# joshloyal/dynetlsm

Measured on AMD Instinct MI355X. Metric: Gibbs iterations/sec (and ms/log-lik eval), T=10 N=2000 d=2, higher is better.
Workload: dtype f64; 1 GPU; DynamicNetworkLSM synthetic undirected T=10 N=2000 d=2, 1 chain per GPU; chains=1, chains_per_gpu=1, sweep_algo=4, network_broadcast=none

## Files before the change

dynetlsm_amd/csrc/capi.hip:

```cpp
#include <hip/hip_runtime.h>
#include <hip/hip_ext.h>

#include <algorithm>
#include <atomic>
#include <cmath>
#include <cstdio>
#include <cstring>
#include <string>
#include <vector>

#include "chain.hpp"
#include "device_common.hpp"
#include "kernels_labels.hpp"
#include "kernels_hdp.hpp"
#include "cc_rows.hpp"
#include "kernels_loglik.hpp"
#include "kernels_loglik_ccstream.hpp"
#include "kernels_hdploop.hpp"
#include "kernels_sweep.hpp"
#include "kernels_dirloop.hpp"
#include "kernels_spec.hpp"
#include "kernels_spec_sweep.hpp"
#include "kernels_spec_pipe.hpp"
#include "kernels_tail_propose.hpp"
#include "kernels_ccpipe.hpp"
#include "kernels_init.hpp"
#include "kernels_post.hpp"
#include "kernels_forecast.hpp"
#include "kernels_forecast_paths.hpp"
#include "kernels_gof.hpp"
#include "kernels_gof_dynamic.hpp"
#include "kernels_ic.hpp"
#include "kernels_score.hpp"
#include "kernels_missing.hpp"
#include "host_draws.hpp"

using namespace dlsm;

static thread_local std::string g_err;
static int32_t *g_fix_err_host = nullptr;
static int g_fix_err_device = -1;
static std::atomic<int> g_live_chains{0};

namespace {

int env_int(const char *name, int unset) { const char *e = getenv(name); return e ? atoi(e) : unset; }
bool env_is(const char *name, const char *word) { const char *e = getenv(name); return e && strcmp(e, word) == 0; }

struct Knobs {
    bool cc_pass_records, cc_pass_rows;
    bool pipe_lds;
    int pipe_xserve, pipe_xbudget;
    int cc_helpers, cc_helper_budget;
    int spec_s;
    bool post_ride, post_fuse, tail_propose, hdp_head;
    bool graph;
    int hdp_queues, hdp_fork_budget;
    bool hdp_gate_kernel;
    bool profiler;
};

Knobs read_knobs() {
    Knobs k;
    k.cc_pass_records = env_is("DLSM_CC_PASS", "records"); k.cc_pass_rows = env_is("DLSM_CC_PASS", "rows");
    k.pipe_lds = env_int("DLSM_PIPE_LDS", 1) != 0;
    k.pipe_xserve = env_int("DLSM_PIPE_XSERVE", 1); k.pipe_xbudget = env_int("DLSM_PIPE_XBUDGET", 1 << 22);
    k.cc_helpers = env_int("DLSM_CC_HELPERS", 1); k.cc_helper_budget = env_int("DLSM_CC_HELPER_BUDGET", 1 << 22);
    k.spec_s = env_int("DLSM_SPEC_S", 2);
    k.post_ride = env_int("DLSM_POST_RIDE", 1) != 0; k.post_fuse = env_int("DLSM_POST_FUSE", 1) != 0;
    k.tail_propose = env_int("DLSM_TAIL_PROPOSE", 1) != 0; k.hdp_head = env_int("DLSM_HDP_HEAD", 1) != 0;
    k.graph = env_int("DLSM_GRAPH", 0) == 1;
    k.hdp_queues = env_int("DLSM_HDP_QUEUES", 0); k.hdp_fork_budget = env_int("DLSM_HDP_FORK_BUDGET", 1 << 22);
    k.hdp_gate_kernel = env_is("DLSM_HDP_GATE", "kernel");
    k.profiler = getenv("ROCP_TOOL_LIBRARIES") != nullptr || getenv("ROCPROFILER_REGISTER_FORCE_LOAD") != nullptr;
    return k;
}

bool labels_wave_forced() {
    static const bool v = env_is("DLSM_LABELS_KERNEL", "wave");
    return v;
}

bool alone_or_forced(int mode, int off, int forced) {
    return mode != off && (mode == forced || g_live_chains.load() == 1);
}

struct Call {
    hipStream_t stream;
    Knobs knobs;
};

struct SweepCall : Call {
    explicit SweepCall(const Call &c) : Call(c) {}
    bool want_post_ride = false; const double *xref = nullptr;
    bool draw_intercept = false, head_only = false, alloc_only = false;
    bool rode = false; int nwg = 0, jl = -1, par = 0;
    bool left_proposals = false;
};

}

#define FAIL(h, code, ...)                                      \
    do {                                                        \
        char _b[512];                                           \
        snprintf(_b, sizeof(_b), __VA_ARGS__);                  \
        if (h) (h)->err = _b; else g_err = _b;                  \
        return (code);                                          \
    } while (0)

#define HIPCHK(h, call)                                                          \
    do {                                                                         \
        hipError_t _e = (call);                                                  \
        if (_e != hipSuccess)                                                    \
            FAIL(h, DLSM_E_HIP, "%s failed: %s (%s:%d)", #call,                  \
                 hipGetErrorString(_e), __FILE__, __LINE__);                     \
    } while (0)

#define NEED(h, cond, ...)                               \
    do {                                                 \
        if (!(cond)) FAIL(h, DLSM_E_ARG, __VA_ARGS__);   \
    } while (0)

#ifdef DLSM_DEV_ONLY_D2
#define DISPATCH_D(h, D_, ...)                                              \
    switch (D_) {                                                           \
        case 2: { constexpr int DD = 2; __VA_ARGS__; } break;               \
        default: FAIL(h, DLSM_E_LIMIT, "n_features=%d: this development build holds n_features = 2 only", D_); \
    }
#else
#define DISPATCH_D(h, D_, ...)                                              \
    switch (D_) {                                                           \
        case 1: { constexpr int DD = 1; __VA_ARGS__; } break;               \
        case 2: { constexpr int DD = 2; __VA_ARGS__; } break;               \
        case 3: { constexpr int DD = 3; __VA_ARGS__; } break;               \
        case 4: { constexpr int DD = 4; __VA_ARGS__; } break;               \
        case 5: { constexpr int DD = 5; __VA_ARGS__; } break;               \
        case 6: { constexpr int DD = 6; __VA_ARGS__; } break;               \
        case 7: { constexpr int DD = 7; __VA_ARGS__; } break;               \
        case 8: { constexpr int DD = 8; __VA_ARGS__; } break;               \
        default: FAIL(h, DLSM_E_LIMIT, "n_features=%d unsupported (1..8)", D_); \
    }
#endif

static int check_pipe_err(dlsm_chain *h);
static int check_sweep_algo(dlsm_chain *h, int algo);
static int build_colmajor(dlsm_chain *h);

static void drop_graph(dlsm_chain *h) {
    if (h->graph_exec) hipGraphExecDestroy(h->graph_exec);
    if (h->graph) hipGraphDestroy(h->graph);
    h->graph_exec = nullptr; h->graph = nullptr; h->graph_ref = -2; h->graph_algo = -1;
}

namespace {

struct ProfScope {
    dlsm_chain *h; int k; hipStream_t q; hipEvent_t e0 = nullptr, e1 = nullptr;
    ProfScope(dlsm_chain *h_, int k_) : ProfScope(h_, k_, h_->stream) {}
    ProfScope(dlsm_chain *h_, int k_, hipStream_t q_) : h(h_), k(k_), q(q_) {
        if (h->profiling) {
            hipEventCreate(&e0); hipEventCreate(&e1);
            hipEventRecord(e0, q);
        }
    }
    ~ProfScope() {
        if (h->profiling) {
            hipEventRecord(e1, q);
            h->prof[k].pending.emplace_back(e0, e1);
        }
    }
};

template <typename T>
int dev_alloc(dlsm_chain *h, T **p, size_t n) {
    HIPCHK(h, hipMalloc((void **)p, std::max<size_t>(n, 1) * sizeof(T)));
    return DLSM_OK;
}

constexpr size_t STAGE_BYTES = 256 * 1024;
constexpr size_t STAGE_D2H_MAX = 64 * 1024;

template <typename T>
int h2d(dlsm_chain *h, T *dst, const T *src, size_t n) {
    const size_t bytes = n * sizeof(T);
    const void *from = src;
    if (h->stage && bytes <= STAGE_BYTES) { memcpy(h->stage, src, bytes); from = h->stage; }
    HIPCHK(h, hipMemcpyAsync(dst, from, bytes, hipMemcpyHostToDevice, h->stream));
    HIPCHK(h, hipStreamSynchronize(h->stream));
    return DLSM_OK;
}

template <typename T>
int d2h(dlsm_chain *h, T *dst, const T *src, size_t n) {
    const size_t bytes = n * sizeof(T);
    const bool staged = h->stage && bytes <= STAGE_D2H_MAX;
    HIPCHK(h, hipMemcpyAsync(staged ? h->stage : (void *)dst, src, bytes, hipMemcpyDeviceToHost,
                             h->stream));
    HIPCHK(h, hipStreamSynchronize(h->stream));
    if (staged) memcpy(dst, h->stage, bytes);
    return DLSM_OK;
}

template <typename T>
int h2d_enqueue(dlsm_chain *h, T *dst, const T *src, size_t n, size_t *off) {
    const size_t bytes = n * sizeof(T);
    const void *from = src;
    if (h->stage && *off + bytes <= STAGE_BYTES) {
        from = (char *)h->stage + *off;
        memcpy((void *)from, src, bytes);
        *off += (bytes + 255) & ~(size_t)255;
    }
    HIPCHK(h, hipMemcpyAsync(dst, from, bytes, hipMemcpyHostToDevice, h->stream));
    return DLSM_OK;
}

int upload_i64_as_i32(dlsm_chain *h, int32_t **dst, const int64_t *src, size_t n,
                      int64_t lo, int64_t hi, const char *what) {
    std::vector<int32_t> tmp(n);
// ... 777 lines not shown
    const size_t TN = (size_t)h->T * h->N;
    rc = ensure_partials(h, TN); if (rc) return rc;
    DISPATCH_D(h, h->D, rc = launch_partial<DD>(h, with_prior, -1, -1, nullptr, h->partials));
    if (rc) return rc;
    return d2h(h, out, h->partials, TN);
}

}


template <int DD, int SBM>
static void launch_spec_eval(dlsm_chain *h, const ChainView &v, const SpecBuf &sg, dim3 grid,
                             hipStream_t q, int parity, int j0, int nsb) {
    hipEvent_t e0 = nullptr, e1 = nullptr;
    if (h->profiling) { hipEventCreate(&e0); hipEventCreate(&e1); }
    if (h->model == DLSM_UNDIRECTED)
        hipExtLaunchKernelGGL((k_spec_eval<DD, DLSM_UNDIRECTED, SBM>), grid, dim3(SP_EV_THREADS),
                              0, q, e0, e1, 0, v, sg, parity, j0, nsb);
    else
        hipExtLaunchKernelGGL((k_spec_eval<DD, DLSM_DIRECTED, SBM>), grid, dim3(SP_EV_THREADS),
                              0, q, e0, e1, 0, v, sg, parity, j0, nsb);
    if (h->profiling) h->prof[DLSM_K_SWEEP_EVAL].pending.emplace_back(e0, e1);
}

template <int DD>
static int launch_sweep_spec(dlsm_chain *h, const SweepCall &sc, IterRef iter, int S) {
    const int N = h->N, T = h->T;
    hipStream_t q = sc.stream;
    if (h->model == DLSM_DIRECTED_CASE_CONTROL) S = 1;
    S = std::max(1, std::min(S, SP_SMAX));
    const int B = std::min(S * SP_BMAX, (N + 1) / 2 * 2);
    const int nsl_max = (T + 1) / 2;
    int parts = (1024 + nsl_max * SP_BMAX - 1) / (nsl_max * SP_BMAX);
    parts = std::max(1, std::min(parts, 8));
    if (h->model == DLSM_DIRECTED_CASE_CONTROL) parts = 1;
    auto even2 = [](size_t n) { return (n + 1) / 2 * 2; };
    const size_t n_full0 = even2((size_t)nsl_max * B * parts);
    const size_t n_prop = even2((size_t)nsl_max * N * (DD + 2));
    const size_t n_ht = (size_t)nsl_max * B * B;
    const size_t need = (n_full0 + n_prop + n_ht + 2) * sizeof(double);
    if (h->spec_cap < need) {
        if (h->spec) hipFree(h->spec);
        h->spec = nullptr; h->spec_cap = 0;
        HIPCHK(h, hipMalloc((void **)&h->spec, need));
        h->spec_cap = need;
    }
    SpecBuf sb;
    sb.full0 = h->spec; sb.prop = sb.full0 + n_full0; sb.Ht = sb.prop + n_prop;
    sb.consts = sb.Ht + n_ht;
    sb.B = B; sb.parts = parts; sb.s0 = 0; sb.per = (N + parts - 1) / parts;
    sb.stamps = nullptr;
    ChainView v = h->view();
    auto resolve = k_spec_resolve<DD>;
    const size_t lds = (size_t)SP_BMAX * SP_BMAX * sizeof(double);
    HIPCHK(h, hipFuncSetAttribute((const void *)resolve,
                                  hipFuncAttributeMaxDynamicSharedMemorySize, (int)lds));
    if (sc.alloc_only) return DLSM_OK;
    for (int parity = 0; parity < 2; ++parity) {
        const int nsl = (T - parity + 1) / 2;
        if (nsl <= 0) continue;
        hipLaunchKernelGGL((k_spec_propose<DD>), dim3((N + 255) / 256, nsl), dim3(256), 0, q, v, sb, iter, parity);
        for (int j0 = 0; j0 < N; j0 += B) {
            const int nsb = std::min(B, N - j0);
            SpecBuf sg = sb;
            const size_t nblk = (size_t)parts * nsb * nsl;
            if (h->profiling && h->stamps && h->model != DLSM_DIRECTED_CASE_CONTROL &&
                h->stamps_used + nblk <= h->stamps_cap) {
                sg.stamps = h->stamps + 2 * h->stamps_used;
                h->stamp_launches.emplace_back(h->stamps_used, nblk);
                h->stamps_used += nblk;
            }
            if (h->model == DLSM_DIRECTED_CASE_CONTROL) {
                ProfScope pe(h, DLSM_K_SWEEP_EVAL, q);
                hipLaunchKernelGGL((k_spec_eval_cc<DD>), dim3((unsigned)(nsl * nsb)),
                                   dim3(64), 0, q, v, sg, h->nctrl, parity, j0, nsb);
            } else if (S == 1)
                launch_spec_eval<DD, SP_BMAX>(h, v, sg, dim3(parts, nsb, nsl), q, parity, j0, nsb);
            else if (S == 2)
                launch_spec_eval<DD, 2 * SP_BMAX>(h, v, sg, dim3(parts, nsb, nsl), q, parity, j0, nsb);
            else
                launch_spec_eval<DD, SP_SMAX * SP_BMAX>(h, v, sg, dim3(parts, nsb, nsl), q, parity, j0, nsb);
            {
                ProfScope pr(h, DLSM_K_SWEEP_RESOLVE, q);
                hipLaunchKernelGGL(resolve, dim3(nsl), dim3(SP_RES_THREADS), lds, q, v, sg, parity, j0, nsb);
            }
        }
    }
    HIPCHK(h, hipGetLastError());
    return DLSM_OK;
}


static int resolve_sweep_algo(const dlsm_chain *h, int algo) {
    if (algo != 0) return algo;
    if (h->D > DLSM_D_PIPE_MAX) return h->N >= 256 ? 2 : 1;
    if (h->model == DLSM_DIRECTED_CASE_CONTROL)
        return (h->N >= 2048 && h->D <= DLSM_D_CCPIPE_MAX) ? 5 : (h->N >= 512 ? 4 : (h->N >= 256 ? 2 : 1));
    return h->N >= 512 ? 4 : (h->N >= 256 ? 2 : 1);
}

template <int DD, int MODEL, int G = 1>
static void launch_pipe_step(dlsm_chain *h, hipStream_t q, const ChainView &v, const PipeBuf &pb, dim3 grid,
                             size_t lds, int l) {
    hipEvent_t e0 = nullptr, e1 = nullptr;
    if (h->profiling) { hipEventCreate(&e0); hipEventCreate(&e1); }
    hipExtLaunchKernelGGL((k_pipe_step<DD, MODEL, G>), grid, dim3(PP_THREADS), lds, q,
                          e0, e1, 0, v, pb, l);
    if (h->profiling) h->prof[DLSM_K_SWEEP_EVAL].pending.emplace_back(e0, e1);
}

static int check_pipe_err(dlsm_chain *h) {
    if (g_fix_err_host && *(volatile int32_t *)g_fix_err_host != 0) {
        const int32_t e = *(volatile int32_t *)g_fix_err_host;
        *(volatile int32_t *)g_fix_err_host = 0;
        FAIL(h, DLSM_E_HIP, "case-control sweep: a resolver's fixed point did not settle inside its spin bound "
             "(word %#x) - the state of this process's case-control chains is undefined; set it again", e);
    }
    if (h->fork_err_host) {
        const int32_t e = *(volatile int32_t *)h->fork_err_host;
        if (e != 0) {
            *(volatile int32_t *)h->fork_err_host = 0;
            if (e & PP_ERR_XSERVE)
                FAIL(h, DLSM_E_HIP, "pipelined sweep: a resolver ran out of its poll budget waiting for a cross product "
                     "from the launch's evaluators (word %#x) - the chain's state is undefined; set the state again "
                     "and run with DLSM_PIPE_XSERVE=0", e);
            if (e & CC_ERR_HELPER)
                FAIL(h, DLSM_E_HIP, "case-control sweep: a resolver ran out of its poll budget waiting for its helper "
                     "workgroup (word %#x) - the chain's state is undefined; set the state again and run with "
                     "DLSM_CC_HELPERS=0", e);
            FAIL(h, DLSM_E_HIP, "HDP-LPCM loop: a hand-over between the chain's two queues ran out of its poll "
                 "budget (flags %d) - the chain's state is undefined (more streams alive than hardware "
                 "queues?); set the state again and run with DLSM_HDP_QUEUES=1", e);
        }
    }
    return DLSM_OK;
}

template <int DD>
static int launch_sweep_pipe(dlsm_chain *h, SweepCall &sc, IterRef iter) {
    constexpr int G = 1;
    hipStream_t q = sc.stream;
    const Knobs &kn = sc.knobs;
    const int N = h->N, T = h->T;
    const int nbat = (N + PP_B - 1) / PP_B;
    const bool cc = h->model == DLSM_DIRECTED_CASE_CONTROL;
    int ne_wg = std::max(h->n_cu / 2, h->n_cu - T);
    int parts = (int)((double)ne_wg * PP_WAVES / ((double)T * PP_B) + 0.5);
    parts = std::max(1, std::min(parts, PP_MAXPARTS));
    if (h->model == DLSM_UNDIRECTED && parts > 1 && (long)parts * T * PP_B > (long)ne_wg * PP_WAVES) --parts;
    if (cc) {
        parts = CC_PARTS;
        ne_wg = std::min(ne_wg, (T * PP_B * CC_PARTS + PP_WAVES - 1) / PP_WAVES);
    }
    auto even2 = [](size_t n) { return (n + 1) / 2 * 2; };
    const size_t n_prop = even2((size_t)T * N * (2 * DD + 2));
    const int xr = (2 * G - 1) * PP_B;
    const size_t n_full0 = (size_t)2 * G * T * PP_B * parts * 2;
    const size_t n_h = (size_t)2 * G * T * PP_B * PP_B;
    const size_t n_hx = (size_t)2 * G * T * xr * PP_B;
    const size_t n_acc = even2(((size_t)T * 2 * G * PP_ACC + 1) / 2);
    const size_t n_xp = (size_t)T * PP_B;
    const size_t need = (n_prop + n_full0 + n_h + n_hx + n_acc + 2 + n_xp) * sizeof(double);
    if (h->pipe_cap < need) {
        if (h->pipe) hipFree(h->pipe);
        h->pipe = nullptr; h->pipe_cap = 0;
        HIPCHK(h, hipMalloc((void **)&h->pipe, need));
        h->pipe_cap = need;
    }
    PipeBuf pb{};
    pb.prop = h->pipe; pb.full0 = pb.prop + n_prop; pb.Hd = pb.full0 + n_full0;
    pb.Hx = pb.Hd + n_h; pb.acc = (int32_t *)(pb.Hx + n_hx);
    pb.consts = pb.Hx + n_hx + n_acc;
    pb.xprod = pb.consts + 2;
    pb.sync = nullptr; pb.nsync = 0; pb.queue0 = ne_wg;
    pb.lsm_draw = sc.draw_intercept ? h->lsm : nullptr;
    pb.parts = parts; pb.nbat = nbat;
    pb.G = G; pb.xr = xr;
    pb.per = ((N + parts - 1) / parts + 63) / 64 * 64;
    pb.nctrl = h->nctrl;
    const size_t lds = (size_t)PP_B * PR_LD * sizeof(double);
    pb.lds_eval = h->model == DLSM_UNDIRECTED && pipe_lds_eval_bytes(N, DD, parts) <= lds &&
                  (long)parts * T * PP_B <= (long)ne_wg * PP_WAVES && kn.pipe_lds;
    pb.err = h->fork_err_dev;
    pb.budget = kn.pipe_xbudget;
    const int xserve_sweep = pb.lds_eval && pb.err != nullptr && T < 128 && alone_or_forced(kn.pipe_xserve, 0, 2);
    pb.xserve = 0;
    ChainView v = h->view();
    {
        PipeLds &a = pb.lds;
        a.X = v.X; a.ybits = v.ybits; a.prop = pb.prop; a.full0 = pb.full0; a.Hd = pb.Hd; a.acc = pb.acc;
        a.consts = pb.consts; a.xprod = pb.xprod;
        a.T = T; a.N = N; a.W = v.W; a.squared = v.squared; a.parts = parts; a.nbat = nbat;
        a.lds_cap = pipe_lds_trip_cap((N + 63) / 64, parts); a.xserve = 0;
    }
    for (int nw = 1; nw <= 4; ++nw)
        for (int p = 0; p < PP_MAXPARTS; ++p)
            pb.lds.plan[nw - 1][p] = p < parts ? pipe_plan_entry((N + 63) / 64, parts, nw, p) : 0u;
    auto ku = k_pipe_step<DD, DLSM_UNDIRECTED>;
    auto kl = k_pipe_step<DD, PIPE_UNDIRECTED_LONG>;
    auto kd = k_pipe_step<DD, DLSM_DIRECTED>;
    auto kc = k_pipe_step<DD, DLSM_DIRECTED_CASE_CONTROL>;
    HIPCHK(h, hipFuncSetAttribute((const void *)ku, hipFuncAttributeMaxDynamicSharedMemorySize,
                                  (int)lds));
    HIPCHK(h, hipFuncSetAttribute((const void *)kl, hipFuncAttributeMaxDynamicSharedMemorySize,
                                  (int)lds));
    HIPCHK(h, hipFuncSetAttribute((const void *)kd, hipFuncAttributeMaxDynamicSharedMemorySize,
                                  (int)lds));
    HIPCHK(h, hipFuncSetAttribute((const void *)kc, hipFuncAttributeMaxDynamicSharedMemorySize,
                                  (int)lds));
    HIPCHK(h, hipFuncSetAttribute((const void *)k_pipe_last_ride<DD>,
                                  hipFuncAttributeMaxDynamicSharedMemorySize, (int)lds));
    if (sc.alloc_only) return DLSM_OK;
    {
        const ProposeBuf nb{pb.prop, pb.consts, pb.sync, pb.nsync, pb.queue0, pb.lsm_draw};
        if (!h->carry.drawn(iter.ptr ? -1L : (long)iter.value, nb))
            hipLaunchKernelGGL((k_pipe_propose<DD>), dim3((N + 255) / 256, T), dim3(256), 0, q, v, pb, iter);
        h->carry.taken(nb); sc.left_proposals = true;
    }
    const int nlaunch = (nbat + G - 1) / G;
    const int last = T > 1 ? nlaunch : nlaunch - 1;
    for (int l = -1; l <= last; ++l) {
        if (l == -1 && !iter.ptr && h->carry.head_done_for == (long)iter.value) continue;
        if (sc.head_only && l >= 0) break;
        const bool any_eval = (G * (l + 1) < nbat) || (T > 1 && l >= 0 && G * l < nbat);
        const int grid = T + (any_eval ? ne_wg : 0);
        const bool lng = !pb.lds_eval;
        if (l == last && !any_eval && sc.want_post_ride && G == 1 && h->model == DLSM_UNDIRECTED &&
            !h->profiling && l >= 0 && T + 4 <= PS_BLOCKS) {
            const long rows = (long)T * N;
            const int nwg = (int)std::min<long>(PS_BLOCKS - T, (rows + PP_THREADS - 1) / PP_THREADS);
            PipePostRide pr{sc.xref, iter, h->partials + (size_t)ll_blocks(h) * 4, nwg,
                            (nbat - 1) * PP_B, T > 1 ? 1 : 0};
            hipLaunchKernelGGL((k_pipe_last_ride<DD>), dim3(T + nwg), dim3(PP_THREADS), lds, q, v, pb, l, pr);
            sc.rode = true; sc.nwg = nwg + T; sc.jl = pr.jl; sc.par = pr.par;
            continue;
        }
        if (h->model == DLSM_UNDIRECTED && lng)
            launch_pipe_step<DD, PIPE_UNDIRECTED_LONG>(h, q, v, pb, dim3(grid), lds, l);
        else if (h->model == DLSM_UNDIRECTED && pb.lds_eval && any_eval) {
            const int beE = l + 1, beO = l, nE = (T + 1) / 2, nO = T / 2;
            PipeLds &a = pb.lds;
            a.beE = beE; a.beO = beO;
            a.nbE = (beE >= 0 && beE < nbat) ? std::min(PP_B, N - beE * PP_B) : 0;
            a.nbO = (beO >= 0 && beO < nbat) ? std::min(PP_B, N - beO * PP_B) : 0;
            a.nslE = a.nbE > 0 ? nE : 0; a.nslO = a.nbO > 0 ? nO : 0;
            const int gx = PP_B / PP_WAVES, nsl = a.nslE + a.nslO;
            a.nsl_magic = (65536u + (uint32_t)nsl - 1u) / (uint32_t)nsl;
            a.xstride = (T * PP_B + ne_wg - 1) / ne_wg;
            pb.xserve = a.xserve = xserve_sweep && a.xstride <= PP_WAVES;
            (void)gx;
            launch_pipe_step<DD, DLSM_UNDIRECTED>(h, q, v, pb, dim3(grid), lds, l);
        } else if (h->model == DLSM_UNDIRECTED)
            launch_pipe_step<DD, DLSM_UNDIRECTED>(h, q, v, pb, dim3(grid), lds, l);
        else if (h->model == DLSM_DIRECTED)
            launch_pipe_step<DD, DLSM_DIRECTED>(h, q, v, pb, dim3(grid), lds, l);
        else
            launch_pipe_step<DD, DLSM_DIRECTED_CASE_CONTROL>(h, q, v, pb, dim3(grid), lds, l);
    }
    HIPCHK(h, hipGetLastError());
    return DLSM_OK;
}

template <int DD>
static int launch_sweep_ccpipe(dlsm_chain *h, SweepCall &sc, IterRef iter) {
    hipStream_t q = sc.stream;
    const int N = h->N, T = h->T;
    const int nbat = (N + CP_B - 1) / CP_B;
    const int cap = std::max(1, h->Din + h->Dout + 2 * h->C);
    auto even2 = [](size_t n) { return (n + 1) / 2 * 2; };
    const size_t n_prop = even2((size_t)T * N * (2 * DD + 2));
    const size_t n_tot = (size_t)2 * T * CP_B;
    const size_t n_ent = (size_t)2 * T * cap * CP_B;
    const size_t n_cnt = (size_t)2 * T * CP_B * 2;
    const size_t n_rec = (size_t)T * N * cp_record_width(DD);
    const size_t n_xsum = (size_t)T * CP_B;
    const size_t need = (n_prop + n_tot + 2 * n_ent + 2 + 2 * n_rec + n_xsum) * sizeof(double) +
                        even2(2 * n_ent + n_cnt) * sizeof(int32_t) +
                        (size_t)T * CP_WAVES * sizeof(unsigned long long);
    if (h->pipe_cap < need) {
        if (h->pipe) hipFree(h->pipe);
        h->pipe = nullptr; h->pipe_cap = 0;
        HIPCHK(h, hipMalloc((void **)&h->pipe, need));
        h->pipe_cap = need;
    }
    if (N >= (1 << 24) || (double)(T + 1) * N * cp_record_width(DD) * sizeof(double) >= 4294967296.0)
        FAIL(h, DLSM_E_LIMIT, "case-control sweep (algo 5): N=%d T=%d is beyond its 32-bit gather offsets "
             "(N < 2^24, (T + 1) N record bytes < 2^32); use sweep_algo 4 or 2", N, T);
    { int rc_ = ensure_cc_rows(h, q, sc.alloc_only); if (rc_) return rc_; }
    const int tw = h->cc_tw;
    if (sc.alloc_only) return DLSM_OK;
    CcPipeBuf pb;
    pb.prop = h->pipe; pb.tot = pb.prop + n_prop; pb.xval = pb.tot + n_tot; pb.oval = pb.xval + n_ent;
    double *consts = pb.oval + n_ent;
    pb.cur = consts + 2; pb.snap = pb.cur + n_rec;
    pb.xsum = pb.snap + n_rec;
    pb.xidx = (int32_t *)(pb.xsum + n_xsum); pb.oidx = pb.xidx + n_ent; pb.cnt = pb.oidx + n_ent;
    pb.accmask = (unsigned long long *)(pb.xidx + even2(2 * n_ent + n_cnt));
    pb.helpers = alone_or_forced(sc.knobs.cc_helpers, 0, 2) && h->n_cu >= 4 * T && h->fork_err_dev != nullptr;
    pb.budget = sc.knobs.cc_helper_budget;
    pb.err = h->fork_err_dev;
    pb.nctrl = h->nctrl; pb.cap = cap; pb.nbat = nbat;
    pb.terms = h->cc_terms; pb.tw = tw;
    PipeBuf pp{};
    pp.prop = pb.prop; pp.consts = consts;
    ChainView v = h->view();
    {
        const ProposeBuf nb{pp.prop, pp.consts, nullptr, 0, 0, nullptr};
        if (!h->carry.drawn(iter.ptr ? -1L : (long)iter.value, nb))
            hipLaunchKernelGGL((k_pipe_propose<DD>), dim3((N + 255) / 256, T), dim3(256), 0, q, v, pp, iter);
        h->carry.taken(nb); sc.left_proposals = true;
    }
    hipLaunchKernelGGL((k_ccpipe_pack<DD>), dim3((unsigned)(((size_t)T * N + 255) / 256)), dim3(256), 0,
                       q, v, pb);
    const int nodes_max = ((T + 1) / 2 + T / 2) * std::min(CP_B, N);
    const int n_front = pb.helpers ? 2 * T : T;
    const int ne_wg = std::max(1, std::min(std::max(h->n_cu / 2, h->n_cu - n_front), nodes_max));
    const int last = T > 1 ? nbat : nbat - 1;
    for (int l = -1; l <= last; ++l) {
        const bool any_eval = (l + 1 < nbat) || (T > 1 && l >= 0 && l < nbat);
        const int grid = n_front + (any_eval ? ne_wg : 0);
        hipEvent_t e0 = nullptr, e1 = nullptr;
        if (h->profiling) { hipEventCreate(&e0); hipEventCreate(&e1); }
        hipExtLaunchKernelGGL((k_ccpipe_step<DD>), dim3(grid), dim3(CP_THREADS), 0, q, e0, e1,
                              0, v, pb, l);
        if (h->profiling) h->prof[DLSM_K_SWEEP_EVAL].pending.emplace_back(e0, e1);
    }
    HIPCHK(h, hipGetLastError());
    return DLSM_OK;
}

template <int DD>
static int launch_sweep(dlsm_chain *h, SweepCall &sc, IterRef iter, int algo) {
    ChainView v = h->view();
    hipStream_t q = sc.stream;
    const bool alloc_only = sc.alloc_only;
    ProfScope ps(h, DLSM_K_SWEEP, q);
    if (h->model == DLSM_DIRECTED_CASE_CONTROL) {
        { int rc_ = ensure_cc_rows(h, q, alloc_only); if (rc_) return rc_; }
        algo = resolve_sweep_algo(h, algo);
        if (alloc_only) hipStreamSynchronize(q);
        if constexpr (DD <= DLSM_D_CCPIPE_MAX) {
            if (algo == 5) return launch_sweep_ccpipe<DD>(h, sc, iter);
        }
        if constexpr (DD <= DLSM_D_PIPE_MAX) {
            if (algo == 4) return launch_sweep_pipe<DD>(h, sc, iter);
        }
        if (algo >= 2) return launch_sweep_spec<DD>(h, sc, iter, 1);
        if (alloc_only) return DLSM_OK;
        for (int parity = 0; parity < 2; ++parity) {
            int nsl = (h->T - parity + 1) / 2;
            if (nsl <= 0) continue;
            hipLaunchKernelGGL((k_sweep_casecontrol<DD>), dim3(nsl), dim3(CC_THREADS), 0,
                               q, v, h->nctrl, iter, parity);
        }
        HIPCHK(h, hipGetLastError());
        return DLSM_OK;
    }
    algo = resolve_sweep_algo(h, algo);
    if constexpr (DD <= DLSM_D_PIPE_MAX) {
        if (algo == 4) return launch_sweep_pipe<DD>(h, sc, iter);
    }
    if (algo == 2) return launch_sweep_spec<DD>(h, sc, iter, 1);
    if (algo == 3) return launch_sweep_spec<DD>(h, sc, iter, sc.knobs.spec_s);
    const size_t lds = sweep_slice_lds_bytes(h->N, DD, h->W, h->model);
    if (lds > 160 * 1024)
        FAIL(h, DLSM_E_LIMIT, "N=%d needs %zu B of LDS in the slice sweep (max 163840)",
             h->N, lds);
    {
        auto ku = k_sweep_slice<DD, DLSM_UNDIRECTED>;
        auto kd = k_sweep_slice<DD, DLSM_DIRECTED>;
        HIPCHK(h, hipFuncSetAttribute((const void *)ku,
                                      hipFuncAttributeMaxDynamicSharedMemorySize, (int)lds));
        HIPCHK(h, hipFuncSetAttribute((const void *)kd,
                                      hipFuncAttributeMaxDynamicSharedMemorySize, (int)lds));
    }
    if (alloc_only) return DLSM_OK;
    for (int parity = 0; parity < 2; ++parity) {
        int nsl = (h->T - parity + 1) / 2;
        if (nsl <= 0) continue;
        if (h->model == DLSM_UNDIRECTED)
            hipLaunchKernelGGL((k_sweep_slice<DD, DLSM_UNDIRECTED>), dim3(nsl), dim3(SW_THREADS),
                               lds, q, v, iter, parity);
        else
            hipLaunchKernelGGL((k_sweep_slice<DD, DLSM_DIRECTED>), dim3(nsl), dim3(SW_THREADS),
                               lds, q, v, iter, parity);
    }
    HIPCHK(h, hipGetLastError());
    return DLSM_OK;
}

static int check_sweep_algo(dlsm_chain *h, int algo) {
    NEED(h, algo >= 0 && algo <= 5, "algo must be 0..5 (6 and 7, measured slower than 4, were removed in round 5)");
    NEED(h, algo != 5 || h->model == DLSM_DIRECTED_CASE_CONTROL, "algo 5 is the case-control sweep");
    NEED(h, algo != 4 || h->D <= DLSM_D_PIPE_MAX, "the pipelined sweep (algo 4) is built for n_features <= 8");
    NEED(h, algo != 5 || h->D <= DLSM_D_CCPIPE_MAX,
         "the sparse case-control sweep (algo 5) is not built for this n_features");
    return DLSM_OK;
}

static int check_ready_sweep(dlsm_chain *h) {
// ... 666 lines not shown
```

dynetlsm_amd/csrc/kernels_spec_pipe.hpp:

```cpp
#pragma once
#include "kernels_spec_sweep.hpp"
#include "kernel_stamps.hpp"

namespace dlsm {

#ifndef DLSM_H_SHIFT
#define DLSM_H_SHIFT 1
#endif
#ifndef DLSM_TRIP_PRIO
#define DLSM_TRIP_PRIO 1
#endif
#if DLSM_TRIP_PRIO
#define DLSM_TRIP_PRIO_STEP(U_)                                                                \
        if ((U_) == 0) __builtin_amdgcn_s_setprio(3);                                          \
        else if ((U_) == (PP_NPRE * 1) / 4) __builtin_amdgcn_s_setprio(2);                     \
        else if ((U_) == (PP_NPRE * 2) / 4) __builtin_amdgcn_s_setprio(1);                     \
        else if ((U_) == (PP_NPRE * 3) / 4) __builtin_amdgcn_s_setprio(0);
#else
#define DLSM_TRIP_PRIO_STEP(U_)
#endif
constexpr int PP_THREADS = 1024;
constexpr int PP_WAVES = PP_THREADS / 64;
constexpr int PP_B = 128;
constexpr int PP_MAXPARTS = 8;
constexpr int PP_ACC = PP_B + 8;
constexpr int PP_ACC_MASK = PP_B + 4;

struct PipeLds {
    const double *X; const uint32_t *ybits; double *prop; double *full0; double *Hd; int32_t *acc; double *consts;
    double *xprod;
    int T, N, W, squared, parts, nbat, lds_cap, xserve;
    int beE, beO, nbE, nbO, nslE, nslO, xstride; uint32_t nsl_magic;
    uint32_t plan[4][8];
};
static_assert(sizeof(PipeLds) == 256, "PipeLds: two 64-byte halves of scalars and the plan table");

struct PipeBuf {
    double *prop;
    double *full0;
    double *Hd;
    double *Hx;
    int32_t *acc;
    double *consts;
    const int32_t *nctrl;
    int parts, per, nbat;
    int G, xr;
    int32_t *sync; int nsync, queue0;
    LsmDeviceState *lsm_draw;
    PipeLds lds;
    double *xprod; int32_t *err; int xserve, budget;
    int lds_eval;
};
constexpr unsigned long long PP_XP_EMPTY = 0x7FF8C0DE5EED0002ull;
constexpr int PP_ERR_XSERVE = 1 << 29;
__host__ __device__ __forceinline__ int pipe_window_start(int b, int G) {
    const int ws = G * (b / G - 1);
    return ws > 0 ? ws : 0;
}

__device__ __forceinline__ void pipe_propose_consts(const ChainView &c, double *consts,
                                                    const double *intercept) {
    const double E = c.model == DLSM_UNDIRECTED ? exp(intercept[0]) : exp(intercept[0] + intercept[1]);
    consts[0] = E;
    consts[1] = (double)flush_interval(E);
}

__device__ __forceinline__ void pipe_propose_intercept(const ChainView &c, LsmDeviceState *lsm,
                                                       const double *intercept, uint32_t iter) {
    double u0, u1, z0, z1;
    philox_uniform2(c.seed, 0, 0, iter, stream_word(c.chain, STREAM_INTERCEPT), u0, u1);
    box_muller(u0, u1, z0, z1);
    const double b0 = intercept[0];
    lsm->cand[0] = b0;
    lsm->cand[1] = b0 + lsm->i_step[0] * z0;
    philox_uniform2(c.seed, 0, 1, iter, stream_word(c.chain, STREAM_INTERCEPT), u0, u1);
    lsm->logu = log(u0);
}

template <int D>
__device__ __forceinline__ void pipe_propose_row_from(const ChainView &c, const ProposeBuf &pb, uint32_t iter,
                                                      int t, int j, const double (&x0)[D]) {
    const int N = c.N;
    double x1[D], logu;
    make_proposal<D>(c, iter, t, j, x0, c.step[(size_t)t * N + j], x1, logu);
    double *pr = pb.prop + ((size_t)t * N + j) * (2 * D + 2);
#pragma unroll
    for (int d = 0; d < D; ++d) { pr[d] = x1[d]; pr[D + 2 + d] = x0[d]; }
    {
        double u0, u1;
        philox_uniform2(c.seed, (uint32_t)j, (uint32_t)t, iter,
                        stream_word(c.chain, STREAM_SWEEP_UNIFORM), u0, u1);
        pr[D] = u0;
    }
    pr[D + 1] = 0.0;
}

template <int D>
__device__ __forceinline__ void pipe_propose_rows(const ChainView &c, const ProposeBuf &pb, uint32_t iter,
                                                  int fb, int tid) {
    const int N = c.N, nbx = (N + 255) / 256;
    const int t = fb / nbx;
    const int j = (fb - t * nbx) * 256 + tid;
    if (pb.sync) {
        const int flat = fb * 256 + tid;
        if (flat < pb.nsync) pb.sync[(size_t)flat * 16] = flat == 0 ? pb.queue0 : 0;
    }
    if (j >= N) return;
    double x0[D], x1[D], logu;
#pragma unroll
    for (int d = 0; d < D; ++d) x0[d] = c.X[((size_t)t * N + j) * D + d];
    make_proposal<D>(c, iter, t, j, x0, c.step[(size_t)t * N + j], x1, logu);
    double *pr = pb.prop + ((size_t)t * N + j) * (2 * D + 2);
#pragma unroll
    for (int d = 0; d < D; ++d) { pr[d] = x1[d]; pr[D + 2 + d] = x0[d]; }
    {
        double u0, u1;
        philox_uniform2(c.seed, (uint32_t)j, (uint32_t)t, iter,
                        stream_word(c.chain, STREAM_SWEEP_UNIFORM), u0, u1);
        pr[D] = u0;
    }
    pr[D + 1] = 0.0;
}

template <int D>
__global__ __launch_bounds__(256) void k_pipe_propose(ChainView c, PipeBuf pb, IterRef ir) {
    const int fb = (int)blockIdx.y * (int)gridDim.x + (int)blockIdx.x;
    if (fb == 0 && threadIdx.x == 0) {
        pipe_propose_consts(c, pb.consts, c.intercept);
        if (pb.lsm_draw) pipe_propose_intercept(c, pb.lsm_draw, c.intercept, ir.get());
    }
    const ProposeBuf nb{pb.prop, pb.consts, pb.sync, pb.nsync, pb.queue0, pb.lsm_draw};
    pipe_propose_rows<D>(c, nb, ir.get(), fb, (int)threadIdx.x);
}


__device__ __forceinline__ double lane_get(double v, int byte_addr) {
    return __hiloint2double(__builtin_amdgcn_ds_bpermute(byte_addr, __double2hiint(v)),
                            __builtin_amdgcn_ds_bpermute(byte_addr, __double2loint(v)));
}
__device__ __forceinline__ void pipe_reduce(double s, double a, double b, int lane, double &sum,
                                            double &ratio) {
    const int x16 = (lane ^ 16) << 2, x32 = (lane ^ 32) << 2;
    s += dpp_move<0xB1>(s);
    a *= dpp_move<0xB1>(a);
    b *= dpp_move<0xB1>(b);
    double q = (lane & 1) ? b : a;
    s += dpp_move<0x4E>(s);
    q *= dpp_move<0x4E>(q);
    s += dpp_move<0x124>(s);
    q *= dpp_move<0x124>(q);
    s += dpp_move<0x128>(s);
    q *= dpp_move<0x128>(q);
    s += lane_get(s, x16);
    q *= lane_get(q, x16);
    s += lane_get(s, x32);
    q *= lane_get(q, x32);
    sum = s;
    ratio = q * fast_rcp(dpp_move<0xB1>(q));
}

#include "kernels_pipe_item.hpp"
#include "kernels_pipe_ccdense.hpp"

constexpr int PR_LD = PP_B + 1;

__device__ __forceinline__ double group8_prod(double v) {
    v *= dpp_move<0xB1>(v);
    v *= dpp_move<0x4E>(v);
    v *= dpp_move<0x141>(v);
    return v;
}
__device__ __forceinline__ double group8_sum(double v) {
    v += dpp_move<0xB1>(v);
    v += dpp_move<0x4E>(v);
    v += dpp_move<0x141>(v);
    return v;
}

template <int D>
__device__ __forceinline__ void row_resolve(const ChainView &c, const PipeBuf &pb, int b, int t,
                                                double *sD, double *sPart,
                                                unsigned long long (*sMask)[2],
                                                double *sCross,
                                                unsigned long long *sSatMask, double *sTab, bool served,
                                                Stamps<PIPE_RES_T> rst) {
    constexpr int PW = 2 * D + 2;
    const int tid = threadIdx.x, lane = tid & 63, wave = tid >> 6;
    DLSM_STAMP(rst, 0, (double)tid)
    const int N = c.N;
    const int j0 = b * PP_B;
    const int nb = min(PP_B, N - j0);
    const int bb = b & 1;
    const int half = wave & 1, part = wave >> 1;
    const int k = 64 * half + lane;
    const bool owner = wave < 2;
    const bool valid = k < nb;
    const double *H = pb.Hd + ((size_t)bb * c.T + t) * PP_B * (2 * PP_B);
    const int kx = tid >> 3, jx = tid & 7;
    double cr[16];
    const uint32_t cr_off = (uint32_t)((kx * (2 * PP_B) + 2 * jx) * sizeof(double));
    if (b > 0 && !served) {
#pragma unroll
        for (int u = 0; u < 8; ++u) {
#if defined(DLSM_X_RES) && (DLSM_X_RES & 1)
            const double2 v = make_double2(1.0, 1.0);
#else
            const double2 v = coh_load2<false>(H, cr_off, (uint32_t)(16 * u * sizeof(double)));
#endif
            cr[2 * u] = v.x; cr[2 * u + 1] = v.y;
        }
    }
    constexpr int BLK_H = D <= 2 ? 8 : 4;
    double2 blk[BLK_H];
    const uint32_t blk_off = (uint32_t)((wave * (2 * PP_B) + PP_B + 2 * lane) * sizeof(double));
#pragma unroll
    for (int u = 0; u < BLK_H; ++u)
#if defined(DLSM_X_RES) && (DLSM_X_RES & 2)
        blk[u] = make_double2(1.0, 1.0);
#else
        blk[u] = coh_load2<false>(H, blk_off, (uint32_t)(u * PP_WAVES * (2 * PP_B) * sizeof(double)));
#endif
    double2 tv[4];
    double x1[D], x0[D], uk = 1.0, st = 0.0;
    int32_t na = 0, ns = 0, un = 0;
    NodePriorPre<D> npre;
    const int kc = min(k, nb - 1);
    const int p1 = pb.parts;
    const double2 *frec = (const double2 *)pb.full0 + ((size_t)bb * c.T + t) * PP_B * pb.parts;
#pragma unroll
    for (int d = 0; d < D; ++d) { x1[d] = 0.0; x0[d] = 0.0; }
#pragma unroll
    for (int u = 0; u < 4; ++u) tv[u] = make_double2(0.0, 1.0);
    auto owner_loads = [&]() {
#pragma unroll
        for (int u = 0; u < 4; ++u)
            tv[u] = coh_load2<false>(frec, (uint32_t)((kc * p1 + min(u, p1 - 1)) * sizeof(double2)));
        const double *pr = pb.prop + ((size_t)t * N + j0 + kc) * PW;
#pragma unroll
        for (int d = 0; d < D; ++d) { x1[d] = pr[d]; x0[d] = pr[D + 2 + d]; }
        uk = pr[D];
        const size_t tjc = (size_t)t * N + j0 + kc;
        st = c.step[tjc]; na = c.nacc[tjc]; ns = c.nsteps[tjc]; un = c.until[tjc];
        npre.request1(c, t, j0 + kc);
    };
    if (owner) owner_loads();
    double tabv = 0.0;
    if (tid < EXPTAB_N) tabv = c_exp2_tab[tid];
#pragma unroll
    for (int u = 0; u < BLK_H; ++u) {
        double *dst = sD + (u * PP_WAVES + wave) * PR_LD + 2 * lane;
        dst[0] = blk[u].x; dst[1] = blk[u].y;
    }
    if (BLK_H < 8) {
        __builtin_amdgcn_sched_barrier(0);
#pragma unroll
        for (int u = 0; u < 8 - BLK_H; ++u)
            blk[u] = coh_load2<false>(H, blk_off, (uint32_t)((BLK_H + u) * PP_WAVES * (2 * PP_B) * sizeof(double)));
#pragma unroll
        for (int u = 0; u < 8 - BLK_H; ++u) {
            double *dst = sD + ((BLK_H + u) * PP_WAVES + wave) * PR_LD + 2 * lane;
            dst[0] = blk[u].x; dst[1] = blk[u].y;
        }
    }
    if (owner) npre.request2(c);
    unsigned int mp = 0u;
    if (b > 0) {
        const unsigned long long *pmg = (const unsigned long long *)(pb.acc + ((size_t)t * 2 + ((b - 1) & 1)) * PP_ACC +
                                                                     PP_ACC_MASK);
        const unsigned long long pm0 = pmg[0], pm1 = pmg[1];
        const unsigned long long mlo = pm0 >> (2 * jx), mhi = pm1 >> (2 * jx);
#pragma unroll
        for (int u = 0; u < 8; ++u)
            mp |= ((unsigned int)((u < 4 ? mlo : mhi) >> (16 * (u & 3))) & 3u) << (2 * u);
        if (!served) {
            double prod = 1.0;
#pragma unroll
            for (int i = 0; i < 16; ++i) prod *= (mp >> i) & 1u ? cr[i] : 1.0;
            const double v = group8_prod(prod);
            if (jx == 0) sCross[kx] = v;
        }
    }
    double r = 0.0, lu = 0.0, lr = 0.0;
    bool sat = false;
    if (owner) {
        double tot = tv[0].x, pr_ = tv[0].y;
#pragma unroll
        for (int u = 1; u < 4; ++u)
            if (u < p1) { tot += tv[u].x; pr_ *= tv[u].y; }
        for (int u = 4; u < p1; ++u) {
            const double2 w = coh_load2<false>(frec, (uint32_t)((kc * p1 + u) * sizeof(double2)));
            tot += w.x; pr_ *= w.y;
        }
        const double prior = npre.value(x1) - npre.value(x0);
        const double ek = tot + prior;
        sat = !(fabs(ek) <= 700.0);
        r = sat ? 1.0 : pr_;
        lr = ek;
        lu = uk;
        if (sat) { lr = ek + log(pr_); lu = log(lu); }
        const unsigned long long sm = __ballot(sat);
        if (lane == 0) sSatMask[half] = sm;
    }
    if (tid < EXPTAB_N) sTab[tid] = tabv;
    __syncthreads();
    if (owner && !sat) r *= tab_exp(lr, sTab);
    DLSM_STAMP(rst, 1, (double)tid)
    const unsigned long long sat0 = sSatMask[0], sat1 = sSatMask[1];
    const bool anysat = (sat0 | sat1) != 0ull;
    const bool satk = (((half ? sat1 : sat0) >> lane) & 1ull) != 0ull;
    if (anysat && b > 0) {
        const bool satx = ((((kx >> 6) ? sat1 : sat0) >> (kx & 63)) & 1ull) != 0ull;
        if (__ballot(satx) != 0ull) {
            double lsum = 0.0;
#pragma unroll
            for (int u = 0; u < 8; ++u) {
                const double2 v = coh_load2<false>(H, cr_off, (uint32_t)(16 * u * sizeof(double)));
                if (satx && ((mp >> (2 * u)) & 1u)) lsum += log(v.x);
                if (satx && ((mp >> (2 * u + 1)) & 1u)) lsum += log(v.y);
            }
            const double vs = group8_sum(lsum);
            if (satx && jx == 0) sCross[kx] = vs;
        }
        __syncthreads();
    }
    if (owner) {
        if (b > 0) {
            double vk;
            if (served && !sat) {
                vk = 1.0;
                if (valid) {
                    const unsigned long long *slotp = (const unsigned long long *)&pb.xprod[(size_t)t * PP_B + k];
                    unsigned long long got = PP_XP_EMPTY;
                    for (int n = 0; n < pb.budget; ++n) {
                        got = __hip_atomic_load(slotp, __ATOMIC_RELAXED, __HIP_MEMORY_SCOPE_AGENT);
                        if (__ballot(got == PP_XP_EMPTY) == 0ull) break;
                        __builtin_amdgcn_s_sleep(1);
                    }
                    if (got == PP_XP_EMPTY)
                        __hip_atomic_fetch_or(pb.err, PP_ERR_XSERVE, __ATOMIC_RELAXED, __HIP_MEMORY_SCOPE_SYSTEM);
                    vk = __longlong_as_double((long long)got);
                    pb.xprod[(size_t)t * PP_B + k] = __longlong_as_double((long long)PP_XP_EMPTY);
                }
            } else {
                if (served && valid)
                    pb.xprod[(size_t)t * PP_B + k] = __longlong_as_double((long long)PP_XP_EMPTY);
                vk = sCross[k];
            }
            if (sat) lr += vk; else r *= vk;
        }
        const unsigned long long g = __ballot(valid && !(sat ? lu >= lr : lu >= r));
        if (lane == 0) sMask[0][half] = g;
    }
    __syncthreads();
    DLSM_STAMP(rst, 2, (double)tid)
    int cur = 0;
    for (int pass = 0; pass < 2 * PP_B + 2; ++pass) {
        const unsigned long long gm = sMask[cur][part >> 2];
        unsigned int bits = (unsigned int)(gm >> (16 * (part & 3))) & 0xFFFFu;
        const int mbase = 16 * part;
        double sum = 1.0, lsum = 0.0;
        if (half == 1 || part < 4) {
            const double *rowk = sD + k * PR_LD;
            while (bits) {
                int f[4];
                double h[4];
#pragma unroll
                for (int u = 0; u < 4; ++u) {
                    f[u] = bits ? mbase + __builtin_ctz(bits) : 1 << 20;
                    bits &= bits - 1u;
                }
#pragma unroll
                for (int u = 0; u < 4; ++u) h[u] = rowk[f[u] < (1 << 20) ? f[u] : 0];
                if (!anysat) {
#pragma unroll
                    for (int u = 0; u < 4; ++u) sum *= k > f[u] ? h[u] : 1.0;
                } else {
#pragma unroll
                    for (int u = 0; u < 4; ++u)
                        if (k > f[u]) { if (satk) lsum += log(h[u]); else sum *= h[u]; }
                }
            }
// ... 221 lines not shown
```

dynetlsm_amd/csrc/pipe_plan.hpp:

```cpp
#pragma once
#include <stdint.h>
#include <stddef.h>
#ifdef __HIPCC__
#define DLSM_PLAN_HD __host__ __device__
#else
#define DLSM_PLAN_HD
#endif

namespace dlsm {

constexpr int PL_EXPTAB_DOUBLES = 2048;

constexpr int PL_WIN = 4;

DLSM_PLAN_HD inline int pipe_lds_trip_cap(int ntrip, int parts) { return (ntrip + parts - 1) / parts + PL_WIN; }
DLSM_PLAN_HD inline size_t pipe_lds_eval_bytes(int N, int D, int parts) {
    const int ntrip = (N + 63) / 64;
    return ((size_t)PL_EXPTAB_DOUBLES + (size_t)(pipe_lds_trip_cap(ntrip, parts) + PL_WIN) * 64 * D) * sizeof(double);
}

struct PipePlan {
    int glo, nwin;
    int w, r, s;
    DLSM_PLAN_HD inline int trips() const { return w + r; }
    DLSM_PLAN_HD inline int trip(int u, int p, int P) const {
        if (u < w) return glo + p + P * u;
        const int rho = s + (u - w);
        return rho < glo ? rho : rho + nwin;
    }
};
inline uint32_t pipe_plan_entry(int ntrip, int P, int nwin, int p) {
    auto wof = [&](int j) { return j < nwin ? (nwin - j + P - 1) / P : 0; };
    const int R = ntrip - nwin, S = R + 2 * nwin;
    const int q = S / P, rem = S % P;
    const bool balanced = R >= 0 && q >= 2 * wof(0);
    const int Rp = R > 0 ? R : 0;
    int s = 0, w = 0, r = 0;
    for (int j = 0; j <= p; ++j) {
        const int wj = wof(j);
        const int rj = balanced ? q + (j < rem ? 1 : 0) - 2 * wj : Rp / P + (j < Rp % P ? 1 : 0);
        if (j < p) s += rj; else { w = wj; r = rj; }
    }
    return (uint32_t)w | ((uint32_t)r << 3) | ((uint32_t)s << 16);
}
DLSM_PLAN_HD inline PipePlan pipe_plan_from_entry(uint32_t e, int ntrip, int be, int k0) {
    PipePlan pl;
    pl.glo = be > 0 ? 2 * be - 2 : 0;
    const int ghi0 = 2 * be + (k0 >= 64 ? 1 : 0);
    const int ghi = ghi0 < ntrip - 1 ? ghi0 : ntrip - 1;
    pl.nwin = ghi - pl.glo + 1;
    pl.w = (int)(e & 7u); pl.r = (int)((e >> 3) & 0x1fffu); pl.s = (int)(e >> 16);
    return pl;
}

}
```

Before: 4903 Gibbs iterations/s.

## Split head pipeline launch across more evaluator parts for even slices

In the pipelined sweep, the head launch (l = -1) evaluates only the even time slices. It can therefore give each slice more evaluator partitions than the steady-state launches do. It allocates a separate record buffer for that head launch and rebuilds the LDS plan entries for the larger part count. The owner kernel then reads the matching record buffer and part count for even slices at l = 0. The aim is to fill idle evaluator waves during the head launch, at the cost of extra buffer space, per-launch plan rebuilding, and a new limit check on the magic divisor.

```diff
diff --git a/dynetlsm_amd/csrc/capi.hip b/dynetlsm_amd/csrc/capi.hip
--- a/dynetlsm_amd/csrc/capi.hip
+++ b/dynetlsm_amd/csrc/capi.hip
@@ -49,7 +49,7 @@
 
 struct Knobs {
     bool cc_pass_records, cc_pass_rows;
-    bool pipe_lds;
+    bool pipe_lds, pipe_head_parts;
     int pipe_xserve, pipe_xbudget;
     int cc_helpers, cc_helper_budget;
     int spec_s;
@@ -63,7 +63,7 @@
 Knobs read_knobs() {
     Knobs k;
     k.cc_pass_records = env_is("DLSM_CC_PASS", "records"); k.cc_pass_rows = env_is("DLSM_CC_PASS", "rows");
-    k.pipe_lds = env_int("DLSM_PIPE_LDS", 1) != 0;
+    k.pipe_lds = env_int("DLSM_PIPE_LDS", 1) != 0; k.pipe_head_parts = env_int("DLSM_PIPE_HEAD_PARTS", 1) != 0;
     k.pipe_xserve = env_int("DLSM_PIPE_XSERVE", 1); k.pipe_xbudget = env_int("DLSM_PIPE_XBUDGET", 1 << 22);
     k.cc_helpers = env_int("DLSM_CC_HELPERS", 1); k.cc_helper_budget = env_int("DLSM_CC_HELPER_BUDGET", 1 << 22);
     k.spec_s = env_int("DLSM_SPEC_S", 2);
@@ -1147,15 +1147,25 @@
         parts = CC_PARTS;
         ne_wg = std::min(ne_wg, (T * PP_B * CC_PARTS + PP_WAVES - 1) / PP_WAVES);
     }
+    const size_t lds = (size_t)PP_B * PR_LD * sizeof(double);
+    const bool lds_eval = h->model == DLSM_UNDIRECTED && pipe_lds_eval_bytes(N, DD, parts) <= lds &&
+                          (long)parts * T * PP_B <= (long)ne_wg * PP_WAVES && kn.pipe_lds;
+    const int head_parts = lds_eval && kn.pipe_head_parts
+                               ? pipe_head_parts((T + 1) / 2, ne_wg, PP_WAVES, PP_B, parts, PP_MAXPARTS) : parts;
+    const bool head_own = head_parts != parts;
+    if (lds_eval && !pipe_nsl_magic_exact(ne_wg, T))
+        FAIL(h, DLSM_E_LIMIT, "pipelined sweep: %d evaluator workgroups of %d slices are beyond the role decode's "
+             "16-bit quotient", ne_wg, T);
     auto even2 = [](size_t n) { return (n + 1) / 2 * 2; };
     const size_t n_prop = even2((size_t)T * N * (2 * DD + 2));
     const int xr = (2 * G - 1) * PP_B;
     const size_t n_full0 = (size_t)2 * G * T * PP_B * parts * 2;
+    const size_t n_head0 = head_own ? (size_t)T * PP_B * head_parts * 2 : 0;
     const size_t n_h = (size_t)2 * G * T * PP_B * PP_B;
     const size_t n_hx = (size_t)2 * G * T * xr * PP_B;
     const size_t n_acc = even2(((size_t)T * 2 * G * PP_ACC + 1) / 2);
     const size_t n_xp = (size_t)T * PP_B;
-    const size_t need = (n_prop + n_full0 + n_h + n_hx + n_acc + 2 + n_xp) * sizeof(double);
+    const size_t need = (n_prop + n_full0 + n_h + n_hx + n_acc + 2 + n_xp + n_head0) * sizeof(double);
     if (h->pipe_cap < need) {
         if (h->pipe) hipFree(h->pipe);
         h->pipe = nullptr; h->pipe_cap = 0;
@@ -1167,15 +1177,15 @@
     pb.Hx = pb.Hd + n_h; pb.acc = (int32_t *)(pb.Hx + n_hx);
     pb.consts = pb.Hx + n_hx + n_acc;
     pb.xprod = pb.consts + 2;
+    double *const head0 = pb.xprod + n_xp;
+    pb.full0_even = pb.full0; pb.parts_even = parts;
     pb.sync = nullptr; pb.nsync = 0; pb.queue0 = ne_wg;
     pb.lsm_draw = sc.draw_intercept ? h->lsm : nullptr;
     pb.parts = parts; pb.nbat = nbat;
     pb.G = G; pb.xr = xr;
     pb.per = ((N + parts - 1) / parts + 63) / 64 * 64;
     pb.nctrl = h->nctrl;
-    const size_t lds = (size_t)PP_B * PR_LD * sizeof(double);
-    pb.lds_eval = h->model == DLSM_UNDIRECTED && pipe_lds_eval_bytes(N, DD, parts) <= lds &&
-                  (long)parts * T * PP_B <= (long)ne_wg * PP_WAVES && kn.pipe_lds;
+    pb.lds_eval = lds_eval;
     pb.err = h->fork_err_dev;
     pb.budget = kn.pipe_xbudget;
     const int xserve_sweep = pb.lds_eval && pb.err != nullptr && T < 128 && alone_or_forced(kn.pipe_xserve, 0, 2);
@@ -1185,12 +1195,16 @@
         PipeLds &a = pb.lds;
         a.X = v.X; a.ybits = v.ybits; a.prop = pb.prop; a.full0 = pb.full0; a.Hd = pb.Hd; a.acc = pb.acc;
         a.consts = pb.consts; a.xprod = pb.xprod;
-        a.T = T; a.N = N; a.W = v.W; a.squared = v.squared; a.parts = parts; a.nbat = nbat;
-        a.lds_cap = pipe_lds_trip_cap((N + 63) / 64, parts); a.xserve = 0;
-    }
-    for (int nw = 1; nw <= 4; ++nw)
-        for (int p = 0; p < PP_MAXPARTS; ++p)
-            pb.lds.plan[nw - 1][p] = p < parts ? pipe_plan_entry((N + 63) / 64, parts, nw, p) : 0u;
+        a.T = T; a.N = N; a.W = v.W; a.squared = v.squared; a.nbat = nbat; a.xserve = 0;
+    }
+    auto set_eval_parts = [&](int P, double *rec) {
+        PipeLds &a = pb.lds;
+        a.parts = P; a.full0 = rec; a.lds_cap = pipe_lds_trip_cap((N + 63) / 64, P);
+        for (int nw = 1; nw <= 4; ++nw)
+            for (int p = 0; p < PP_MAXPARTS; ++p)
+                a.plan[nw - 1][p] = p < P ? pipe_plan_entry((N + 63) / 64, P, nw, p) : 0u;
+    };
+    set_eval_parts(parts, pb.full0);
     auto ku = k_pipe_step<DD, DLSM_UNDIRECTED>;
     auto kl = k_pipe_step<DD, PIPE_UNDIRECTED_LONG>;
     auto kd = k_pipe_step<DD, DLSM_DIRECTED>;
@@ -1220,6 +1234,8 @@
         const bool any_eval = (G * (l + 1) < nbat) || (T > 1 && l >= 0 && G * l < nbat);
         const int grid = T + (any_eval ? ne_wg : 0);
         const bool lng = !pb.lds_eval;
+        const bool head_rec = head_own && l == 0;
+        pb.full0_even = head_rec ? head0 : pb.full0; pb.parts_even = head_rec ? head_parts : parts;
         if (l == last && !any_eval && sc.want_post_ride && G == 1 && h->model == DLSM_UNDIRECTED &&
             !h->profiling && l >= 0 && T + 4 <= PS_BLOCKS) {
             const long rows = (long)T * N;
@@ -1235,12 +1251,15 @@
         else if (h->model == DLSM_UNDIRECTED && pb.lds_eval && any_eval) {
             const int beE = l + 1, beO = l, nE = (T + 1) / 2, nO = T / 2;
             PipeLds &a = pb.lds;
+            if (head_own) {
+                if (l == -1) set_eval_parts(head_parts, head0); else if (l == 0) set_eval_parts(parts, pb.full0);
+            }
             a.beE = beE; a.beO = beO;
             a.nbE = (beE >= 0 && beE < nbat) ? std::min(PP_B, N - beE * PP_B) : 0;
             a.nbO = (beO >= 0 && beO < nbat) ? std::min(PP_B, N - beO * PP_B) : 0;
             a.nslE = a.nbE > 0 ? nE : 0; a.nslO = a.nbO > 0 ? nO : 0;
             const int gx = PP_B / PP_WAVES, nsl = a.nslE + a.nslO;
-            a.nsl_magic = (65536u + (uint32_t)nsl - 1u) / (uint32_t)nsl;
+            a.nsl_magic = pipe_nsl_magic(nsl);
             a.xstride = (T * PP_B + ne_wg - 1) / ne_wg;
             pb.xserve = a.xserve = xserve_sweep && a.xstride <= PP_WAVES;
             (void)gx;
diff --git a/dynetlsm_amd/csrc/kernels_spec_pipe.hpp b/dynetlsm_amd/csrc/kernels_spec_pipe.hpp
--- a/dynetlsm_amd/csrc/kernels_spec_pipe.hpp
+++ b/dynetlsm_amd/csrc/kernels_spec_pipe.hpp
@@ -50,6 +50,7 @@
     PipeLds lds;
     double *xprod; int32_t *err; int xserve, budget;
     int lds_eval;
+    double *full0_even; int parts_even;
 };
 constexpr unsigned long long PP_XP_EMPTY = 0x7FF8C0DE5EED0002ull;
 constexpr int PP_ERR_XSERVE = 1 << 29;
@@ -225,8 +226,9 @@
     int32_t na = 0, ns = 0, un = 0;
     NodePriorPre<D> npre;
     const int kc = min(k, nb - 1);
-    const int p1 = pb.parts;
-    const double2 *frec = (const double2 *)pb.full0 + ((size_t)bb * c.T + t) * PP_B * pb.parts;
+    const bool ev = (t & 1) == 0;
+    const int p1 = ev ? pb.parts_even : pb.parts;
+    const double2 *frec = (const double2 *)(ev ? pb.full0_even : pb.full0) + ((size_t)bb * c.T + t) * PP_B * p1;
 #pragma unroll
     for (int d = 0; d < D; ++d) { x1[d] = 0.0; x0[d] = 0.0; }
 #pragma unroll
diff --git a/dynetlsm_amd/csrc/pipe_plan.hpp b/dynetlsm_amd/csrc/pipe_plan.hpp
--- a/dynetlsm_amd/csrc/pipe_plan.hpp
+++ b/dynetlsm_amd/csrc/pipe_plan.hpp
@@ -18,6 +18,14 @@
     const int ntrip = (N + 63) / 64;
     return ((size_t)PL_EXPTAB_DOUBLES + (size_t)(pipe_lds_trip_cap(ntrip, parts) + PL_WIN) * 64 * D) * sizeof(double);
 }
+
+inline int pipe_head_parts(int n_even, int n_wg, int waves, int batch, int parts, int maxparts) {
+    int hp = (int)(((long)n_wg * waves) / ((long)(n_even > 0 ? n_even : 1) * batch));
+    if (hp > maxparts) hp = maxparts;
+    return hp > parts ? hp : parts;
+}
+inline uint32_t pipe_nsl_magic(int nsl) { return (65536u + (uint32_t)nsl - 1u) / (uint32_t)nsl; }
+inline bool pipe_nsl_magic_exact(int n_wg, int nsl) { return nsl >= 1 && (long)((n_wg + 7) / 8) * nsl <= 65536; }
 
 struct PipePlan {
     int glo, nwin;
diff --git a/profiles/pipe_head_ab.py b/profiles/pipe_head_ab.py
--- /dev/null
+++ b/profiles/pipe_head_ab.py
@@ -0,0 +1,37 @@
+import json
+import os
+import sys
+import time
+
+import numpy as np
+import torch
+
+sys.path.insert(0, os.path.dirname(os.path.dirname(os.path.abspath(__file__))))
+from dynetlsm_amd import Chain, SamplerGrid
+from dynetlsm_amd.synthetic import synthetic_lsm_network
+
+T, N, D, STEPS = 10, 2000, 2, 200
+net = synthetic_lsm_network(T, N, D, density=0.03, seed=0)
+ch = Chain(T, N, D, 'undirected', seed=20240229, chain_id=0, device=0)
+ch.upload_network(net['Y'])
+ch.set_positions(net['X_init'])
+ch.set_intercepts([float(net['intercept'])])
+ch.set_prior_random_walk(2.0, 0.1)
+ch.set_samplers(SamplerGrid(T, N, step_size=0.1, tune=None))
+ch.lsm_configure([float(net['intercept'])], 2.0, step_size_intercept=0.1, tune=None, n_iter_procrustes=0,
+                 sweep_algo=4)
+ch.trace_alloc(2 + 300 + 4 * STEPS, logp0=0.0)
+it = 1
+ch.lsm_run(it, 300, procrustes_ref=0); ch.synchronize(); it += 300
+out = []
+for rep in range(2):
+    for mode in ('0', '1'):
+        os.environ['DLSM_PIPE_HEAD_PARTS'] = mode
+        t0 = time.perf_counter()
+        ch.lsm_run(it, STEPS, procrustes_ref=0); ch.synchronize()
+        sec = time.perf_counter() - t0
+        it += STEPS
+        out.append({'head_parts': mode, 'it_per_s': round(STEPS / sec, 1)})
+        print(json.dumps(out[-1]), flush=True)
+for mode in ('0', '1'):
+    print('switch %s: median %.1f it/s' % (mode, np.median([o['it_per_s'] for o in out if o['head_parts'] == mode])))
diff --git a/profiles/pipe_head_durations.py b/profiles/pipe_head_durations.py
--- /dev/null
+++ b/profiles/pipe_head_durations.py
@@ -0,0 +1,16 @@
+import csv
+import sys
+
+import numpy as np
+
+rows = list(csv.DictReader(open(sys.argv[1])))
+rows.sort(key=lambda r: int(r['Start_Timestamp']))
+head, rest, prev_pipe = [], [], False
+for r in rows:
+    pipe = 'k_pipe_step' in r['Kernel_Name']
+    if pipe:
+        (rest if prev_pipe else head).append((int(r['End_Timestamp']) - int(r['Start_Timestamp'])) / 1e3)
+    prev_pipe = pipe
+for name, d in (('head launch (l = -1)', np.array(head)), ('other k_pipe_step launches', np.array(rest))):
+    print('%-28s n %6d  median %6.2f us  mean %6.2f us  p10 %6.2f  p90 %6.2f'
+          % (name, d.size, np.median(d), d.mean(), np.percentile(d, 10), np.percentile(d, 90)))
```

Result: no change. 4946 Gibbs iterations/s (median of 6 runs) (+0.9%).
